# gio54321/quill-zkvm

Hardware: AMD Instinct MI355X
Metric: G1 MSM scalars/sec at 2^24 + sumcheck-prover ms at 2^20 vars (1/8 GPU) (higher is better)
Workload: dtype u256-montgomery (BN254 Fr scalars, Fq coordinates); 1 GPU; KZG commit / Pippenger G1 MSM, 2^24 BN254 scalars per GPU; parallelism=msm-shard-by-base-index x1

## Files before the change

### quill-zkvm_amd/csrc/msm.hip

```cpp
#include <stdlib.h>
#include <string.h>

#include "common.h"
#include "curve29.h"
#include "msm_plan.h"

using namespace qg;

namespace qg {

static constexpr int MSM_BLOCK = 256;

static int msm_window_bits(size_t n) {
  int best = 4;
  double best_cost = 1e300;
  for (int c = 4; c <= 22; c++) {
    const int W = (255 + c - 1) / c;
    const int k = 254 - c * (W - 1);
    if (k < 30 && (n >> k) > 4096) continue;
    const double cost = (double)n * W + 12.0 * (double)((size_t)1 << (c - 1));
    if (cost < best_cost) {
      best_cost = cost;
      best = c;
    }
// ... 724 lines not shown
    if (bstart[mid] <= e0) lo = mid;
    else hi = mid;
  }
  uint32_t b = lo;
  uint32_t next = bstart[b + 1];
  X29 acc;
  bool inf = true;
  if constexpr (PF) {
  uint4 g0 = msm_entries4(entries, e0, e1);
  uint4 g1 = e0 + 4 < e1 ? msm_entries4(entries, e0 + 4, e1) : g0;
  Q29 ax, ay;
#ifndef QG_MSM_ROWMASK
#define QG_MSM_ROWMASK 0x7fffffffu
#endif
  bool pinf = msm_pt_load(table, g0.x & QG_MSM_ROWMASK, (g0.x >> 31) != 0u, ax, ay);
  for (uint32_t e = e0; e < e1; e++) {
    const uint32_t k = e & 3u;
    Q29 bx = ax, by = ay;
    bool qinf = true;
    if (e + 1 < e1) {
      const uint32_t en = k == 0 ? g0.y : k == 1 ? g0.z : k == 2 ? g0.w : g1.x;
      qinf = msm_pt_load(table, en & QG_MSM_ROWMASK, (en >> 31) != 0u, bx, by);
    }
    if (k == 3) {
      g0 = g1;
      if (e + 5 < e1) g1 = msm_entries4(entries, e + 5, e1);
    }
    if (e == next) {
      msm_flush(partial, owner, msm_chunk_of(e1 - 1, Lm) + b, b, acc, inf);
      inf = true;
      do {
        b++;
        next = bstart[b + 1];
      } while (next <= e);
    }
    if (!pinf) {
      if (inf) {
        acc.X = ax;
        acc.Y = ay;
        acc.ZZ = Q29::from_l9(F29P<FqP>::ONE);
        acc.ZZZ = acc.ZZ;
        inf = false;
      } else if (!x29_acc_madd_tp(acc, ax, ay)) {
        x29_acc_madd_exc(acc, ax, ay, &inf);
      }
    }
    ax = bx;
    ay = by;
    pinf = qinf;
  }
  msm_flush(partial, owner, msm_chunk_of(e1 - 1, Lm) + b, b, acc, inf);
  return;
  }
  uint4 cur = msm_entries4(entries, e0, e1), nxt = cur;
  for (uint32_t e = e0; e < e1; e++) {
    const uint32_t k = e & 3u;
    if (k == 0 && e + 4 < e1) nxt = msm_entries4(entries, e + 4, e1);
    const uint32_t ent = k == 0 ? cur.x : k == 1 ? cur.y : k == 2 ? cur.z : cur.w;
    if (k == 3) cur = nxt;
    if (e == next) {
      msm_flush(partial, owner, msm_chunk_of(e1 - 1, Lm) + b, b, acc, inf);
      inf = true;
      do {
        b++;
        next = bstart[b + 1];
      } while (next <= e);
    }
    Q29 ax, ay;
    const bool pinf = msm_pt_load(table, ent & 0x7fffffffu, (ent >> 31) != 0u, ax, ay);
    if (pinf) continue;
    if (inf) {
      acc.X = ax;
      acc.Y = ay;
      acc.ZZ = Q29::from_l9(F29P<FqP>::ONE);
      acc.ZZZ = acc.ZZ;
      inf = false;
      continue;
    }
    if (!x29_acc_madd_tp(acc, ax, ay)) x29_acc_madd_exc(acc, ax, ay, &inf);
  }
  msm_flush(partial, owner, msm_chunk_of(e1 - 1, Lm) + b, b, acc, inf);
}

typedef __attribute__((address_space(3))) void* msm_lds_ptr;
typedef __attribute__((address_space(1))) void* msm_glb_ptr;

#if defined(__HIP_DEVICE_COMPILE__)
__device__ __forceinline__ void msm_coop_issue(uint4* wbuf, const MsmPt* __restrict__ table,
                                               uint32_t lane, uint32_t ent) {
  const uint32_t pos = lane & 7u;
  const uint32_t word = pos ^ ((lane >> 3) & 7u);
  uint32_t r[8];
#pragma unroll
  for (int k = 0; k < 8; k++) r[k] = (uint32_t)__shfl((int)(ent & 0x7fffffffu), 8 * k + (int)(lane >> 3), 64);
  uint32_t rowb = (uint32_t)sizeof(MsmPt);
  asm("" : "+s"(rowb));
  const uint64_t col = (uint64_t)(reinterpret_cast<const uint4*>(table) + word);
#pragma unroll
  for (int k = 0; k < 8; k++) {
    const uint64_t g = (uint64_t)r[k] * rowb + col;
    __builtin_amdgcn_global_load_lds((msm_glb_ptr)g, (msm_lds_ptr)(wbuf + 64 * k), 16, 0, 0);
  }
}

__device__ __forceinline__ bool msm_coop_read(const uint4* wbuf, uint32_t lane, bool neg, Q29& x,
                                              Q29& y) {
  const uint4* row = wbuf + 8 * lane;
  const uint32_t sw = lane & 7u;
  const uint32_t wy = neg ? 4u : 2u;
  const uint4 x0 = row[0u ^ sw], x1 = row[1u ^ sw];
  const uint4 y0 = row[wy ^ sw], y1 = row[(wy + 1u) ^ sw];
  const uint4 top = row[6u ^ sw];
  x.l[0] = x0.x; x.l[1] = x0.y; x.l[2] = x0.z; x.l[3] = x0.w;
  x.l[4] = x1.x; x.l[5] = x1.y; x.l[6] = x1.z; x.l[7] = x1.w;
  y.l[0] = y0.x; y.l[1] = y0.y; y.l[2] = y0.z; y.l[3] = y0.w;
  y.l[4] = y1.x; y.l[5] = y1.y; y.l[6] = y1.z; y.l[7] = y1.w;
  x.l[8] = top.x;
  y.l[8] = neg ? top.z : top.y;
  return (top.w & 1u) != 0u;
}
#endif

__global__ void __launch_bounds__(MSM_BLOCK) __attribute__((amdgpu_waves_per_eu(QG_COOP_WPE)))
    k_msm_accumulate_coop(const MsmPt* __restrict__ table, const uint32_t* __restrict__ entries,
                          const uint32_t* __restrict__ bstart, uint32_t nb, uint32_t L, uint64_t Lm,
                          X29Raw* __restrict__ partial, uint32_t* __restrict__ owner) {
#if defined(__HIP_DEVICE_COMPILE__)
  __shared__ uint4 img[MSM_BLOCK / 64][64 * 8];
  const uint32_t t = blockIdx.x * blockDim.x + threadIdx.x;
  const uint32_t lane = threadIdx.x & 63u;
  uint4* wbuf = img[__builtin_amdgcn_readfirstlane(threadIdx.x >> 6)];
  const uint32_t total = bstart[nb];
  const uint64_t e0w = (uint64_t)t * L;
  if (__builtin_amdgcn_readfirstlane((uint32_t)(e0w >= total))) return;
  const uint32_t e0 = e0w < total ? (uint32_t)e0w : total;
  const uint32_t e1 = total - e0 < L ? total : e0 + L;
  uint32_t b = 0, next = 0;
  if (e0 < e1) {
    uint32_t lo = 0, hi = nb;
    while (hi - lo > 1) {
      const uint32_t mid = (lo + hi) >> 1;
      if (bstart[mid] <= e0) lo = mid;
      else hi = mid;
    }
    b = lo;
    next = bstart[b + 1];
  }
  X29 acc = x29_inf();
  bool inf = true;
  uint4 g0 = msm_entries4(entries, e0, e1);
  uint4 g1 = e0 + 4 < e1 ? msm_entries4(entries, e0 + 4, e1) : g0;
  msm_coop_issue(wbuf, table, lane, e0 < e1 ? g0.x : 0u);
  for (uint32_t i = 0; i < L; i++) {
    const uint32_t e = e0 + i;
    const uint32_t k = i & 3u;
    const uint32_t ent = g0.x;
    asm volatile("s_waitcnt vmcnt(0)" ::: "memory");
    Q29 ax, ay;
    const bool pinf = msm_coop_read(wbuf, lane, (ent >> 31) != 0u, ax, ay);
    asm volatile("s_waitcnt lgkmcnt(0)" ::: "memory");
    if (k == 3) {
      g0 = g1;
      if (e + 5 < e1) g1 = msm_entries4(entries, e + 5, e1);
    } else {
      g0.x = g0.y;
      g0.y = g0.z;
      g0.z = g0.w;
    }
    const uint32_t en = g0.x;
    if (i + 1 < L) msm_coop_issue(wbuf, table, lane, e + 1 < e1 ? en : 0u);
    if (e >= e1) continue;
    if (e == next) {
      if (inf) x29_acc_inf_ip(acc);
      x29_pin(acc);
      msm_flush(partial, owner, msm_chunk_of(e1 - 1, Lm) + b, b, acc, false);
      inf = true;
      do {
        b++;
        next = bstart[b + 1];
      } while (next <= e);
    }
    if (pinf) continue;
    uint32_t add = inf ? 0u : 1u;
    asm("" : "+v"(add));
    if (inf) {
      x29_acc_start_ip(acc, ax, ay);
      inf = false;
    }
    x29_pin(acc);
    if (add) x29_acc_madd_ip(acc, ax, ay, inf);
  }
  if (e0 < e1) msm_flush(partial, owner, msm_chunk_of(e1 - 1, Lm) + b, b, acc, inf);
#endif
}

QG_DEV uint32_t msm_slot_first(const uint32_t* bstart, uint32_t b, uint32_t L) {
  return bstart[b] / L + b;
}
QG_DEV uint32_t msm_slot_last(const uint32_t* bstart, uint32_t b, uint32_t L) {
  return (bstart[b + 1] - 1) / L + b;
}

QG_DEV uint32_t msm_slot_stride(uint32_t nslot, uint32_t T) {
  uint32_t st = 1;
  while (nslot > T * st) st <<= 1;
  return st;
}

__global__ void __launch_bounds__(MSM_BLOCK)
    k_msm_tree_step(X29Raw* __restrict__ partial, const uint32_t* __restrict__ owner,
                    const uint32_t* __restrict__ bstart, uint32_t L, uint32_t T, uint32_t s_lo,
                    uint32_t s_end, uint32_t s, uint32_t* hv, uint32_t gen) {
  msm_handover_check(hv, 2, 2, gen, 2u);
  const uint32_t i = s_lo + blockIdx.x * blockDim.x + threadIdx.x;
  if (i >= s_end) return;
  const uint32_t b = owner[i];
  if (b == 0xffffffffu) return;
  const uint32_t f = msm_slot_first(bstart, b, L), l = msm_slot_last(bstart, b, L);
  if (l - f + 1 <= T * s) return;
  const uint32_t off = i - f;
  if ((off & (2 * s - 1)) == 0 && i + s <= l)
    partial[i] = x29_raw(x29_add(msm_partial(partial, i), msm_partial(partial, i + s)));
}

struct MsmRed {
  const X29Raw* partial;
  const uint32_t* bstart;
  uint32_t L, T;
};
constexpr uint32_t MSM_RED_BYVAL = 8;
struct MsmRedSet {
  MsmRed r[MSM_RED_BYVAL];
};

#if defined(__HIP_DEVICE_COMPILE__)
__device__ __forceinline__ Q29 q29_shfl_down(const Q29& a, uint32_t d, int width) {
  Q29 r;
#pragma unroll
  for (int i = 0; i < 9; i++) r.l[i] = __shfl_down(a.l[i], d, width);
  return r;
}
__device__ __forceinline__ X29 x29_shfl_down(const X29& p, uint32_t d, int width) {
  return {q29_shfl_down(p.X, d, width), q29_shfl_down(p.Y, d, width),
          q29_shfl_down(p.ZZ, d, width), q29_shfl_down(p.ZZZ, d, width)};
}

template <bool Q4>
__device__ __forceinline__ X29 red_add(const X29& a, const X29& b) {
  if constexpr (Q4) return x29_add_q4(a, b);
  else return x29_add(a, b);
}
template <bool Q4>
__device__ __forceinline__ X29 red_dbl(const X29& a) {
  if constexpr (Q4) return x29_dbl_q4(a);
  else return x29_dbl(a);
}

template <bool Q4>
__device__ __forceinline__ void msm_fold(X29& A, X29 Y, int gl, uint32_t mv, int flog, int ylog,
                                         X29& Yw) {
  constexpr uint32_t ES = Q4 ? 4 : 1;
  const int width = (int)(ES << gl);
  const uint32_t g = ((threadIdx.x & 63u) % (uint32_t)width) / ES;
  int ns = 0;
  while ((1u << ns) < mv) ns++;
  X29 Yd = Y;
  for (int s = 0; s < 2 * ns + 1; s++) {
    if (s == ns) {
      Yw = Y;
      Yd = Y;
      X29 t = Y;
      const int nd = flog > ylog ? flog : ylog;
      for (int i = 1; i <= nd; i++) {
        t = red_dbl<Q4>(t);
        if (i == flog) Yd = t;
        if (i == ylog) Yw = t;
      }
    }
    uint32_t d;
    bool live;
    X29 a, o;
    if (s < ns) {
      d = 1u << s;
      o = x29_shfl_down(Y, d * ES, width);
      a = Y;
      live = g + d < mv;
    } else if (s == ns) {
      o = Yd;
      a = A;
      live = g != 0 && g < mv;
    } else {
      d = (1u << ns) >> (s - ns);
      o = x29_shfl_down(A, d * ES, width);
      a = A;
      live = g < d;
    }
    const X29 r = red_add<Q4>(a, x29_sel(live, o, x29_inf()));
    if (s < ns) Y = r;
    else A = r;
  }
}
#endif

__global__ void __launch_bounds__(MSM_BLOCK)
    k_msm_bsum(const MsmRed* __restrict__ runs, MsmRedSet rs, uint32_t nb, int slog, int gl,
               G1Xyzz* __restrict__ A_out, G1Xyzz* __restrict__ Y_out, size_t ostride,
               uint32_t* hv, uint32_t gen) {
#if defined(__HIP_DEVICE_COMPILE__)
  msm_handover_check(hv, 2, 2, gen, 2u);
  const uint32_t t = blockIdx.x * blockDim.x + threadIdx.x;
  const MsmRed rr = runs ? runs[blockIdx.y] : rs.r[blockIdx.y];
  X29 run = x29_inf(), wsum = x29_inf(), B = x29_inf();
  const uint64_t lo64 = (uint64_t)t << slog;
  const uint32_t lo = lo64 < nb ? (uint32_t)lo64 : nb;
  uint32_t j = nb - lo < (1u << slog) ? nb : lo + (1u << slog);
  int stage = 0;
  uint32_t slot = 0, last = 0, step = 1;
  for (;;) {
    if (stage == 0) {
      if (j == lo) break;
      j--;
      const uint32_t s0 = rr.bstart[j], s1 = rr.bstart[j + 1];
      if (s0 == s1) {
        B = x29_inf();
        stage = 2;
      } else {
        const uint32_t f = s0 / rr.L + j;
        last = (s1 - 1) / rr.L + j;
        B = msm_partial(rr.partial, f);
        step = msm_slot_stride(last - f + 1, rr.T);
        slot = f + step;
        stage = slot <= last ? 1 : 2;
      }
    }
    X29 a, b;
    if (stage == 1) {
      a = B;
      b = msm_partial(rr.partial, slot);
    } else {
      a = stage == 2 ? run : wsum;
      b = stage == 2 ? B : run;
    }
    const X29 r = x29_add(a, b);
    if (stage == 1) {
      B = r;
      slot += step;
      if (slot > last) stage = 2;
    } else if (stage == 2) {
      run = r;
      stage = 3;
    } else {
      wsum = r;
      stage = 0;
    }
  }
  X29 Yw;
  msm_fold<false>(wsum, run, gl, 1u << gl, slog, gl + slog, Yw);
  if ((t & ((1u << gl) - 1)) == 0) {
    const size_t w = (size_t)blockIdx.y * ostride + (t >> gl);
    A_out[w] = x29_store(wsum);
    Y_out[w] = x29_store(Yw);
  }
#endif
}

QG_DEV G1Xyzz x29_export_xyzz(const X29& p) {
  if (x29_is_inf(p)) return G1Xyzz::infinity();
  return {q29_export(p.X), q29_export(p.Y), q29_export(p.ZZ), q29_export(p.ZZZ)};
}

template <bool Q4>
__global__ void __launch_bounds__(64)
    k_msm_wfold(const G1Xyzz* __restrict__ A_in, const G1Xyzz* __restrict__ Y_in, uint32_t m,
                size_t istride, G1Xyzz* __restrict__ A_out, G1Xyzz* __restrict__ Y_out,
                size_t ostride) {
#if defined(__HIP_DEVICE_COMPILE__)
  constexpr uint32_t ES = Q4 ? 4 : 1, G = 64 / ES;
  const uint32_t e0 = blockIdx.x * G, e = e0 + threadIdx.x / ES;
  const uint32_t mv = m - e0 < G ? m - e0 : G;
  X29 A = x29_inf(), Y = x29_inf();
  if (e < m) {
    A = x29_load(A_in[(size_t)blockIdx.y * istride + e]);
    Y = x29_load(Y_in[(size_t)blockIdx.y * istride + e]);
  }
  const int gl = Q4 ? 4 : 6;
  X29 Yw;
  msm_fold<Q4>(A, Y, gl, mv, 0, Y_out ? gl : 0, Yw);
  if (threadIdx.x == 0) {
    const size_t w = (size_t)blockIdx.y * ostride + blockIdx.x;
    if (Y_out) {
      A_out[w] = x29_store(A);
      Y_out[w] = x29_store(Yw);
    } else {
      A_out[w] = x29_export_xyzz(A);
    }
  }
#endif
}

__global__ void k_srs_pack(const G1Affine* __restrict__ pts, size_t n, MsmPt* __restrict__ out) {
  const size_t i = (size_t)blockIdx.x * blockDim.x + threadIdx.x;
  if (i >= n) return;
  const G1Affine w = pts[i];
  out[i] = w.is_inf() ? msm_pt_pack(Q29::zero(), Q29::zero(), true)
                      : msm_pt_pack(q29_import(w.x), q29_import(w.y), false);
}

__global__ void k_srs_unpack(const MsmPt* __restrict__ rows, size_t n, G1Affine* __restrict__ out) {
  const size_t i = (size_t)blockIdx.x * blockDim.x + threadIdx.x;
  if (i >= n) return;
  Q29 x, y;
  if (msm_pt_unpack(rows[i], x, y)) {
    out[i] = G1Affine::infinity();
    return;
  }
  out[i] = {q29_export(x), q29_export(y)};
}

__global__ void k_srs_shift(MsmPt* table, size_t N, int w, int c) {
  const size_t i = (size_t)blockIdx.x * blockDim.x + threadIdx.x;
  if (i >= N) return;
  A29 a;
  if (msm_pt_unpack(table[(size_t)(w - 1) * N + i], a.x, a.y)) {
    table[(size_t)w * N + i] = msm_pt_pack(Q29::zero(), Q29::zero(), true);
    return;
  }
  X29 p = x29_from_affine(a);
  for (int k = 0; k < c; k++) p = x29_dbl(p);
  const Q29 t = inv29(mul29(p.ZZ, p.ZZZ));
  const Q29 zzinv = mul29(t, p.ZZZ), zzzinv = mul29(t, p.ZZ);
  table[(size_t)w * N + i] = msm_pt_pack(canon29(mul29(p.X, zzinv)), canon29(mul29(p.Y, zzzinv)),
                                         false);
}

__global__ void k_powers(Fr tau, uint64_t offset, size_t n, int K, Fr* out) {
  size_t t = (size_t)blockIdx.x * blockDim.x + threadIdx.x;
  size_t i0 = t * (size_t)K;
  if (i0 >= n) return;
  Fr x = fpow_small(tau, offset + (uint64_t)i0);
  for (int j = 0; j < K && i0 + j < n; j++) {
    out[i0 + j] = x;
    x = x * tau;
  }
}

__global__ void k_fb_powers(G1Affine g, G1Xyzz* bases) {
  if (threadIdx.x != 0 || blockIdx.x != 0) return;
  G1Xyzz p = G1Xyzz::from_affine(g);
  for (int k = 0; k < 32; k++) {
    bases[k] = p;
    for (int d = 0; d < 8; d++) p = xyzz_dbl(p);
  }
}

__global__ void k_fb_table(const G1Xyzz* __restrict__ bases, G1Affine* __restrict__ fb) {
  int idx = blockIdx.x * blockDim.x + threadIdx.x;
  if (idx >= 32 * 256) return;
  int k = idx >> 8, j = idx & 255;
  G1Xyzz acc = xyzz_mul_small(bases[k], (uint32_t)j);
  fb[idx] = xyzz_to_affine(acc);
}

__global__ void k_fb_mul(const G1Affine* __restrict__ fb, const Fr* __restrict__ scal, size_t n,
                         G1Affine* __restrict__ out) {
  size_t i = (size_t)blockIdx.x * blockDim.x + threadIdx.x;
  if (i >= n) return;
  Fr s = from_mont(scal[i]);
  G1Xyzz acc = G1Xyzz::infinity();
  for (int k = 0; k < 32; k++) {
    uint32_t byte = (s.v[k >> 2] >> (8 * (k & 3))) & 255u;
    if (byte) acc = xyzz_add_affine(acc, fb[k * 256 + byte]);
  }
  out[i] = xyzz_to_affine(acc);
}

__global__ void k_import_bases(const uint64_t* __restrict__ xy, const uint8_t* __restrict__ inf,
                               size_t n, G1Affine* __restrict__ out) {
  size_t i = (size_t)blockIdx.x * blockDim.x + threadIdx.x;
  if (i >= n) return;
  G1Affine a;
  for (int l = 0; l < 4; l++) {
    uint64_t x = xy[8 * i + l], y = xy[8 * i + 4 + l];
    a.x.v[2 * l] = (uint32_t)x;
    a.x.v[2 * l + 1] = (uint32_t)(x >> 32);
    a.y.v[2 * l] = (uint32_t)y;
    a.y.v[2 * l + 1] = (uint32_t)(y >> 32);
  }
  if (inf && inf[i]) a = G1Affine::infinity();
  out[i] = a;
}

void srs_build_tables(qg_ctx* ctx, qg_srs* srs, const G1Affine* base) {
  QgTimed tm(ctx, "srs_shift");
  hipLaunchKernelGGL(k_srs_pack, dim3(div_up(srs->n, 256)), dim3(256), 0, ctx->stream, base,
                     srs->n, srs->d_table);
  QG_LAUNCH_CHECK();
  for (int w = 1; w < srs->tables; w++) {
    hipLaunchKernelGGL(k_srs_shift, dim3(div_up(srs->n, 256)), dim3(256), 0, ctx->stream,
                       srs->d_table, srs->n, w, srs->c);
    QG_LAUNCH_CHECK();
  }
}

qg_srs* srs_alloc(qg_ctx* ctx, size_t n, bool oneshot) {
  qg_srs* srs = new qg_srs();
  srs->ctx = ctx;
  srs->n = n;
  int ct = msm_window_bits(n);
  if (oneshot) ct = std::min(ct, 18);
  if (const char* ov = getenv("QG_MSM_WINDOW_BITS")) ct = atoi(ov);
  QG_CHECK(ct >= 4 && ct <= 26, QG_ERR_INVALID, "MSM window bits out of range");
  srs->W = (255 + ct - 1) / ct;
  srs->c = (255 + srs->W - 1) / srs->W;
  srs->tables = oneshot ? 1 : srs->W;
  hipError_t e = hipMalloc(&srs->d_table, (size_t)srs->tables * n * sizeof(MsmPt));
  if (e != hipSuccess) {
    delete srs;
    throw Error(QG_ERR_OOM, "qg_srs: hipMalloc of the window tables failed");
  }
  return srs;
}

void srs_unpack_rows(qg_ctx* ctx, const qg_srs* srs, size_t offset, size_t n, G1Affine* d_out) {
  hipLaunchKernelGGL(k_srs_unpack, dim3(div_up(n, 256)), dim3(256), 0, ctx->stream,
                     srs->d_table + offset, n, d_out);
  QG_LAUNCH_CHECK();
}

struct MsmRun {
  bool empty = true;
  uint32_t L = 1, T = 4;
  size_t nslots = 0;
  X29Raw* partial = nullptr;
  uint32_t* owner = nullptr;
  uint32_t* bstart = nullptr;
  uint32_t* misc = nullptr;
  uint32_t* h_mx = nullptr;
  hipEvent_t ev_mx = nullptr;
  uint32_t gen = 0;
};
static constexpr int MSM_MAX_BATCH = 1024;

struct MsmJob {
  const Fr* d_scalars = nullptr;
  size_t n = 0;
  int slot = 0;
  size_t srs_off = 0;
  hipStream_t stream = nullptr;
  uint32_t* hv = nullptr;
  uint32_t hgen = 0;
  int wsel = -1;
  bool canon_ready = false;
};

static bool msm_on_side_stream(const qg_ctx* ctx, const MsmJob& job) {
  return job.stream != nullptr && job.stream != ctx->stream;
}

struct SortFn {
  const void* fn;
  std::string key;
};
template <int BLK, bool PF>
static SortFn sortA_fn() {
  return {reinterpret_cast<const void*>(&k_sortA_scatter<BLK, PF>),
          "msm_sortA" + std::to_string(BLK) + (PF ? "pf" : "")};
}
template <int BLK, int CHUNK, bool PF>
static SortFn sortB_fn() {
  return {reinterpret_cast<const void*>(&k_sortB_scatter<BLK, CHUNK, PF>),
          "msm_sortB" + std::to_string(BLK) + "_" + std::to_string(CHUNK) + (PF ? "pf" : "")};
}

static void sort_lds_attr(qg_ctx* ctx, const SortFn& f) {
  const std::string key = f.key + "_lds";
  if (ctx->memo.count(key)) return;
  QG_HIP(hipFuncSetAttribute(f.fn, hipFuncAttributeMaxDynamicSharedMemorySize, 160 * 1024));
  ctx->memo[key] = "1";
}

static int sort_pf_occupancy(qg_ctx* ctx, char pass, int blk, size_t smem) {
  QG_CHECK(blk == 1024, QG_ERR_ASSERT, "the prefetching scatters have 1024 threads");
  const SortFn f = pass == 'A' ? sortA_fn<1024, true>() : sortB_fn<1024, 16384, true>();
  sort_lds_attr(ctx, f);
  const std::string mk = f.key + "_occ" + std::to_string(smem);
  auto it = ctx->memo.find(mk);
  if (it != ctx->memo.end()) return std::stoi(it->second);
  int occ = 0;
  QG_HIP(hipOccupancyMaxActiveBlocksPerMultiprocessor(&occ, f.fn, blk, smem));
  ctx->memo[mk] = std::to_string(occ);
  return occ;
}

static MsmPlan msm_job_plan(qg_ctx* ctx, const qg_srs* srs, const MsmJob& job) {
  const int W = srs->W, wsel = job.wsel;
  QG_CHECK((wsel < 0) == (srs->tables == W) && wsel < W, QG_ERR_INVALID,
           "MSM window selection does not match the SRS tables");
  QG_CHECK((size_t)W * srs->n < 0x80000000ull, QG_ERR_UNSUPPORTED, "SRS table index overflow");
  QG_CHECK(job.slot >= 0 && job.slot < MSM_MAX_BATCH, QG_ERR_UNSUPPORTED, "MSM batch too large");
  MsmShape sh;
  sh.n = job.n;
  sh.c = srs->c;
  sh.W = W;
  sh.wsel = wsel;
  sh.side = msm_on_side_stream(ctx, job);
  sh.cus = ctx->num_cus();
  return msm_plan(sh, msm_tuning_from_env(), [ctx](char pass, int blk, size_t smem) {
    return sort_pf_occupancy(ctx, pass, blk, smem);
  });
}

struct MsmScratch {
  uint32_t *ghist, *goff, *gtiles, *gstart, *cbase, *cgroup;
  uint32_t* misc;
  uint32_t *chist, *coff, *tmp_e;
  uint16_t* tmp_l;
  uint32_t *hrow, *orow;
  Fr* canon;
  uint32_t *counts, *bstart, *entries;
  uint2* tile_tot;
  X29Raw* partial;
  uint32_t* owner;
};

static MsmScratch msm_scratch(qg_ctx* ctx, const MsmPlan& p, size_t n, int slot, bool side,
                              bool run) {
  const std::string sfx = "#" + std::to_string(slot);
  const std::string tg = side ? "@" + std::to_string(slot & 1) : std::string();
  constexpr bool RESERVED = true, RUN_ONLY = false;
  auto get = [&](auto*& ptr, const std::string& name, size_t count, bool reserved) {
    using T = std::remove_reference_t<decltype(*ptr)>;
    if (run || reserved) ptr = ctx->scratch_as<T>(name, count);
  };
  MsmScratch s{};
  get(s.ghist, "msm_ghist" + tg, p.nghist + 1, RESERVED);
  get(s.goff, "msm_goff" + tg, p.nghist + 1, RESERVED);
  get(s.gtiles, "msm_gtiles" + tg, div_up(p.nghist, 2048) + 1, RESERVED);
  get(s.gstart, "msm_gstart" + tg, p.H + 1, RESERVED);
  get(s.cbase, "msm_cbase" + tg, p.H + 1, RESERVED);
  get(s.cgroup, "msm_cgroup" + tg, p.max_chunks, RESERVED);
  get(s.misc, "msm_misc" + sfx, 5, RESERVED);
  get(s.chist, "msm_chist" + tg, p.max_chunks * p.NL, RESERVED);
  get(s.coff, "msm_coff" + tg, p.max_chunks * p.NL, RESERVED);
  get(s.tmp_e, "msm_tmp_e" + tg, p.max_entries + 1, RESERVED);
  get(s.tmp_l, "msm_tmp_l" + tg, p.max_entries + 1, RESERVED);
  get(s.hrow, "msm_hrow" + tg, p.nghist + 1, RESERVED);
  get(s.orow, "msm_orow" + tg, p.nghist + 1, RESERVED);
  get(s.canon, "msm_canon" + tg, n, RESERVED);
  get(s.counts, "msm_counts" + tg, p.nb, RESERVED);
  get(s.bstart, "msm_bstart" + sfx, p.nb + 1, RESERVED);
  get(s.entries, "msm_entries" + tg, p.max_entries + 1, RESERVED);
  get(s.tile_tot, "msm_tiles" + tg, p.ntiles, RUN_ONLY);
  get(s.partial, "msm_partial" + sfx, p.nslots, RUN_ONLY);
  get(s.owner, "msm_owner" + sfx, p.nslots, RUN_ONLY);
  return s;
}
// ... 876 lines not shown
```

Baseline: 985.4 million scalars/s.

## Software-pipeline bucket-sum partial and bstart loads across point additions

```diff
diff --git a/quill-zkvm_amd/csrc/msm.hip b/quill-zkvm_amd/csrc/msm.hip
--- a/quill-zkvm_amd/csrc/msm.hip
+++ b/quill-zkvm_amd/csrc/msm.hip
@@ -1050,6 +1050,10 @@
 }
 #endif
 
+typedef uint32_t quad_t __attribute__((ext_vector_type(4)));
+typedef const quad_t __attribute__((address_space(1)))* GlobalQuads;
+typedef const uint32_t __attribute__((address_space(1)))* GlobalWords;
+
 __global__ void __launch_bounds__(MSM_BLOCK)
     k_msm_bsum(const MsmRed* __restrict__ runs, MsmRedSet rs, uint32_t nb, int slog, int gl,
                G1Xyzz* __restrict__ A_out, G1Xyzz* __restrict__ Y_out, size_t ostride,
@@ -1062,44 +1066,94 @@
   const uint64_t lo64 = (uint64_t)t << slog;
   const uint32_t lo = lo64 < nb ? (uint32_t)lo64 : nb;
   uint32_t j = nb - lo < (1u << slog) ? nb : lo + (1u << slog);
+  const GlobalQuads part = (GlobalQuads)(uintptr_t)rr.partial;
+  const GlobalWords bst = (GlobalWords)(uintptr_t)rr.bstart;
+  const uint32_t L = rr.L, T = rr.T;
+  X29Raw nraw = {};
+  uint32_t w0 = 0, w1 = 0, w2 = 0, wnext = 0, nidx = 0;
+  uint32_t slot = 0, last = 0, step = 1;
+  auto load_raw = [&](quad_t (&q)[9]) {
+#pragma unroll
+    for (int k = 0; k < 9; k++) q[k] = part[(size_t)nidx * 9 + k];
+  };
+  auto take_raw = [&](const quad_t (&q)[9]) {
+#pragma unroll
+    for (int k = 0; k < 9; k++) nraw.q[k] = make_uint4(q[k].x, q[k].y, q[k].z, q[k].w);
+  };
+  auto bst_ahead = [&]() { return bst[j >= lo + 3 ? j - 3 : lo]; };
+  auto start_bucket = [&](uint32_t jn) -> int {
+    bool more = false;
+    if (w1 == w0) {
+      B = x29_inf();
+    } else {
+      const uint32_t f = w1 / L + jn;
+      last = (w0 - 1) / L + jn;
+      B = x29_acc_finish(x29_unraw(nraw));
+      step = msm_slot_stride(last - f + 1, T);
+      slot = f + step;
+      more = slot <= last;
+    }
+    if (more) nidx = slot;
+    else if (jn > lo && w2 != w1) nidx = w2 / L + jn - 1;
+    w0 = w1;
+    w1 = w2;
+    w2 = wnext;
+    return more ? 1 : 2;
+  };
   int stage = 0;
-  uint32_t slot = 0, last = 0, step = 1;
-  for (;;) {
-    if (stage == 0) {
-      if (j == lo) break;
-      j--;
-      const uint32_t s0 = rr.bstart[j], s1 = rr.bstart[j + 1];
-      if (s0 == s1) {
-        B = x29_inf();
-        stage = 2;
-      } else {
-        const uint32_t f = s0 / rr.L + j;
-        last = (s1 - 1) / rr.L + j;
-        B = msm_partial(rr.partial, f);
-        step = msm_slot_stride(last - f + 1, rr.T);
-        slot = f + step;
-        stage = slot <= last ? 1 : 2;
-      }
-    }
+  if (j > lo) {
+    w0 = bst[j];
+    w1 = bst[j - 1];
+    w2 = bst[j >= lo + 2 ? j - 2 : lo];
+    wnext = bst_ahead();
+    if (w1 != w0) nidx = w1 / L + j - 1;
+    quad_t q[9];
+    load_raw(q);
+    take_raw(q);
+    j--;
+    stage = start_bucket(j);
+    load_raw(q);
+    take_raw(q);
+    wnext = bst_ahead();
+  }
+  while (stage != 0) {
     X29 a, b;
+    int nstage = 0;
     if (stage == 1) {
       a = B;
-      b = msm_partial(rr.partial, slot);
+      b = x29_acc_finish(x29_unraw(nraw));
+      slot += step;
+      if (slot <= last) nidx = slot;
+      else if (j > lo && w1 != w0) nidx = w1 / L + j - 1;
+    } else if (stage == 2) {
+      a = run;
+      b = B;
     } else {
-      a = stage == 2 ? run : wsum;
-      b = stage == 2 ? B : run;
-    }
+      a = wsum;
+      b = run;
+      if (j > lo) {
+        j--;
+        nstage = start_bucket(j);
+      }
+    }
+    quad_t q[9];
+    load_raw(q);
+    uint32_t wq = bst_ahead();
+    asm volatile("" ::: "memory");
     const X29 r = x29_add(a, b);
+    asm volatile("" : "+v"(q[0]), "+v"(q[1]), "+v"(q[2]), "+v"(q[3]), "+v"(q[4]), "+v"(q[5]),
+                      "+v"(q[6]), "+v"(q[7]), "+v"(q[8]), "+v"(wq));
+    take_raw(q);
+    wnext = wq;
     if (stage == 1) {
       B = r;
-      slot += step;
       if (slot > last) stage = 2;
     } else if (stage == 2) {
       run = r;
       stage = 3;
     } else {
       wsum = r;
-      stage = 0;
+      stage = nstage;
     }
   }
   X29 Yw;
```

Result: no change. 985.9 million scalars/s, median of 4 (+0.1%).
